# choutilin/makani

Measured on AMD Instinct MI355X. Metric: SFNO fwd+bwd samples/sec, 73ch 721x1440, higher is better.
Workload: dtype bf16; 1 GPU; sfno_linear_73chq_sc3_layers8_edim384 fwd+bwd+Adam, 73ch 721x1440, per-GPU batch 1; global_batch=1, parallelism=h1, spectral_dtype=f32 (GEMMs as 6 bf16 MFMA products of exact 3-way operand splits), step_launch=eager, micro_batches=1, python_gc=disabled in the timed region, adam=after backward

## Files before the change

include/makani_amd.h:

```cpp
#ifndef MAKANI_AMD_H
#define MAKANI_AMD_H

#include <stdint.h>

#ifdef __cplusplus
extern "C" {
#endif

int mk_version(void);
const char* mk_last_error(void);


int mk_quadrature(int grid, int nlat, double* theta, double* weights);

int mk_legendre_kpad(int nlat);

int mk_legendre_table(int grid, int nlat, int lmax, int mmax, int with_quad_weights, float* out);

int mk_fft_twiddle_len(int nlon);
int mk_fft_twiddles(int nlon, float* out);

int mk_rfft(const void* x, int x_dtype, float* xf, const float* twiddles,
            int bc, int nlat, int nlon, int mmax, float scale0, float scale_m, float scale_h,
            void* stream);
// ... 66 lines not shown
int mk_spec_mix_wgrad(const float* x, const float* gy, float* gw, int lloc, int mloc, int batch,
                      int cin, int cout, int l_off, int m_off, void* stream);

int mk_spec_cmlp_fwd(const float* x, const float* w, const float* bias, float* y, int lloc, int mloc, int batch, int cin,
                     int cout, int l_off, int m_off, int per_degree, int act, void* stream);
int mk_spec_cmlp_dgrad(const float* gy, const float* w, const float* a, float* gx, int lloc, int mloc, int batch, int cin,
                       int cout, int l_off, int m_off, int per_degree, int act, void* stream);
long long mk_spec_cmlp_wgrad_workspace(int lloc, int cin, int cout, int per_degree);
int mk_spec_cmlp_wgrad(const float* x, const float* gy, float* gw, void* workspace, int lloc, int mloc, int batch, int cin,
                       int cout, int l_off, int m_off, int per_degree, void* stream);
long long mk_spec_cmlp_bgrad_workspace(int lloc, int cout);
int mk_spec_cmlp_bgrad(const float* g, float* gb, void* workspace, int lloc, int mloc, int batch, int cout, int l_off,
                       int m_off, void* stream);

int mk_spec_bdmlp_fwd(const float* x, const float* w, float* y, int rows, int nb, int ib, int ob, int act, float lambda,
                      void* stream);
int mk_spec_bdmlp_dgrad(const float* gy, const float* w, const float* a, float* gx, int rows, int nb, int ib, int ob, int act,
                        void* stream);
long long mk_spec_bdmlp_wgrad_workspace(int rows, int nb, int ib, int ob);
int mk_spec_bdmlp_wgrad(const float* x, const float* gy, float* gw, void* workspace, int rows, int nb, int ib, int ob,
                        void* stream);
int mk_spec_bdmlp_mask(const float* gy, const float* s, float* out, long long n, void* stream);
int mk_spec_bdmlp_fwd_bias(const float* x, const float* w, const float* bias, float* y, int rows, int nb, int ib, int ob, int act,
                           float lambda, void* stream);

int mk_diag_fwd(const float* x, const float* w, float* y, int batch, int cin, int cout, long long P, void* stream);
int mk_diag_dgrad(const float* gy, const float* w, float* gx, int batch, int cin, int cout, long long P, void* stream);
int mk_diag_wgrad(const float* x, const float* gy, float* gw, int batch, int cin, int cout, long long P, void* stream);

int mk_spec_diag_fwd(const float* x, const float* w, float* y, int lloc, int mloc, int batch,
                     int cin, int cout, int l_off, int m_off, int dense, void* stream);
int mk_spec_diag_dgrad(const float* gy, const float* w, float* gx, int lloc, int mloc, int batch,
                       int cin, int cout, int l_off, int m_off, int dense, void* stream);
int mk_spec_diag_wgrad(const float* x, const float* gy, float* gw, int lloc, int mloc, int batch,
                       int cin, int cout, int l_off, int m_off, int dense, void* stream);

int mk_spec_pack(const float* c_std, float* c_prv, int bc, int lloc, int mloc, void* stream);
int mk_spec_unpack(const float* c_prv, float* c_std, int bc, int lloc, int mloc,
                   int l_off, int m_off, void* stream);
int mk_tokens_to_fields(const void* tok, void* fld, int dtype, int batch, int n, int c, void* stream);
int mk_fields_to_tokens(const void* fld, const void* addend, void* tok, int dtype, int batch, int n, int c, void* stream);
int mk_patch_tile_info(int C, int H, int W, int p0, int p1, int order, long long ldt, int* tile);
int mk_patchify(const void* img, int img_dtype, void* tok, int tok_dtype, long long ldt, int batch, int C, int H, int W, int p0,
                int p1, int order, void* stream);
int mk_unpatchify(const void* tok, int tok_dtype, long long ldt, void* img, int img_dtype, int batch, int C, int H, int W, int p0,
                  int p1, int order, void* stream);

int mk_bias_gelu_fwd(const void* x, const float* bias, void* y, int dtype, int rows, int C, long long P,
                     void* stream);
int mk_bias_gelu_bwd(const void* x, const float* bias, const void* gy, void* gx, float* gbias, int dtype,
                     int rows, int C, long long P, void* stream);
int mk_affine_add(const void* r, const void* z, const float* affine, void* y, int dtype, int rows, long long P,
                  void* stream);
int mk_instnorm_fwd(const void* x, const float* weight, const float* bias, void* y, float* stats,
                    double* workspace, int dtype, int rows, int C, long long P, float eps, int fuse_gelu,
                    void* stream);
int mk_instnorm_bwd(const void* x, const void* gy, const float* stats, const float* weight, const float* bias,
                    void* gx, double* workspace, int dtype, int rows, int C, long long P, int fuse_gelu,
                    void* stream);

int mk_instnorm_fwd_ex(const void* x, const float* weight, const float* bias, void* y, float* stats,
                       double* workspace, int dtype, int rows, int C, long long P, long long count, float eps,
                       int fuse_gelu, int phase, void* stream);
int mk_instnorm_bwd_ex(const void* x, const void* gy, const float* stats, const float* weight, const float* bias,
                       void* gx, double* workspace, int dtype, int rows, int C, long long P, long long count,
                       int fuse_gelu, int phase, void* stream);
int mk_instnorm_bwd_wb(const void* x, const void* gy, const float* stats, const float* weight, const float* bias, void* gx,
                       double* workspace, float* gwb, int dtype, int C, long long P, int fuse_gelu, void* stream);

int mk_wmse_fwd(const void* pred, int dtype, const float* tar, const float* wrow, double* loss, long long rows,
                int H, int W, float scale, void* stream);
int mk_wmse_bwd(const void* pred, int dtype, const float* tar, const float* wrow, const float* gloss, void* gpred,
                long long rows, int H, int W, float scale, void* stream);

int mk_conv1x1_x3(const float* a, long long lda, const float* b, long long ldb, float* c, long long ldc, int M, int K, long long N,
                  int batch, long long sa, long long sb, long long sc, int mode, void* stream);
int mk_conv1x1_x3_bias_act(const float* a, long long lda, const float* b, long long ldb, float* c, long long ldc, int M, int K,
                           long long N, int batch, long long sb, long long sc, const float* bias, int act, void* stream);

int mk_conv1x1_wgrad(const void* gy, const void* x, float* gw, int batch, int cout, int cin, long long P,
                     void* stream);
int mk_conv1x1_wgrad_act(const void* gy, const void* x, float* gw, int batch, int cout, int cin, long long P, int x_act,
                         void* stream);
long long mk_pce_image_bytes(int M, int K);
int mk_pce_pack(const void* w, int w_dtype , int transpose, int M, int K, int ldw, void* img,
                void* stream);
int mk_pce_pack_layout(int M, int K, long long* out3);
int mk_pce_pack_batch(const void* desc_dev, int n, void* arena, long long total_elements, void* stream);
int mk_pce_gemm(const void* x, const void* wimg, void* y, const float* bias, const void* addend, const void* aux_in,
                void* aux_out, int gelu, int batch, int M, int K, long long P, void* stream);
int mk_pce_gemm_ex(const void* x, const void* wimg, void* y, const float* bias, const void* addend, const float* addend_affine,
                   const void* aux_in, void* aux_out, int gelu, double* rowstats, int batch, int M, int K, long long P,
                   void* stream);
long long mk_pce_mlp_image_bytes(int M, int Hd, int K1);
int mk_pce_mlp_pack(const void* a1, int a1_transposed, int lda1, const void* a2, int a2_transposed, int lda2,
                    int w_dtype , int M, int Hd, int K1, void* img, void* stream);
int mk_pce_mlp(const void* x, const void* wimg, void* y, void* mid_out, const void* mid_in, const float* b1, const float* b2,
               double* rowstats_y, double* rowsum_mid, int mode, int batch, int M, int Hd, int K1, long long P, void* stream);
int mk_pce_mlp_debug_stamps(unsigned long long* out512);
int mk_instnorm_coeffs(const double* sums, const float* weight, const float* bias, float* stats, float* affine, int rows,
                       int C, long long count, float eps, void* stream);
int mk_pce_debug_stamps(unsigned long long* out512);

int mk_adam_step(float* p, const float* g, float* m, float* v, long long n, float lr, float beta1, float beta2, float eps,
                 float weight_decay, int step, void* stream);

long long mk_mt_chunks(long long n);
int mk_mt_sumsq(int T, const uint64_t* x, const long long* n, double* partials, double* tsum, int clip_mode, float max_norm,
                float* norm_out, float* coef_out, float* steps, const int* inc_slots, int ninc, void* stream);
int mk_mt_norm_finish(int T, const double* tsum, int clip_mode, float max_norm, float* norm_out, float* coef_out,
                      float* steps, const int* inc_slots, int ninc, void* stream);
int mk_mt_step_inc(float* steps, const int* slots, int nslots, void* stream);
int mk_mt_scale(int T, const uint64_t* x, const long long* n, const float* coef, void* stream);
int mk_mt_adam(int T, const uint64_t* pgmv, const long long* n, const int* step_or_slot, const float* steps, float lr,
               const float* lr_dev, float beta1, float beta2, float eps, float weight_decay, int adamw, const float* coef,
               void* stream);
int mk_mt_lamb(int stage, int T, const uint64_t* pgmv, const long long* n, const int* step_or_slot, const float* steps,
               float lr, const float* lr_dev, float beta1, float beta2, float beta3, float eps, float weight_decay, int adamw,
               int bias_correction, int trust, const float* coef, double* part_p, double* part_u, double* tsum_p,
               double* tsum_u, void* stream);

long long mk_geo_metric_workspace(int B, int C, int H);
int mk_geo_metric_sums(const void* pred, int dtype, const float* tar, const float* clim, const float* wrow, double* workspace,
                       double* sums, int B, int C, int H, int W, void* stream);

long long mk_geo_lp_workspace(int B, int C, int H);
int mk_geo_lp_sums(const void* pred, int dtype, const float* tar, const float* wrow, double* workspace, double* sums, int p,
                   int B, int C, int H, int W, void* stream);
int mk_geo_lp_bwd(const void* pred, int dtype, const float* tar, const float* wrow, const float* g, void* gpred, int p,
                  int B, int C, int H, int W, void* stream);

int mk_input_assemble(const void* x, int x_dtype, const float* u, const float* stat, const float* mean, const float* std,
                      const int* mask_chans, int n_mask, int mask_src, void* out, int out_dtype, int B, int T, int C, int Cu,
                      int Cs, int H, int W, void* stream);
int mk_input_assemble_bwd(const void* gout, int g_dtype, const float* stat, const float* std, const int* mask_chans, int n_mask,
                          int mask_src, void* gx, int x_dtype, int B, int T, int C, int Cu, int Cs, int H, int W, void* stream);

long long mk_history_workspace(int B, int Cn, int H);
int mk_history_sums(const void* x, int x_dtype, const float* u, const float* wt, double* workspace, double* sums, int B, int T,
                    int C, int Cu, int H, int W, void* stream);

long long mk_rollout_tail_workspace(int B, int C, int H);
int mk_rollout_tail(const void* yn, int dtype, const float* mean, const float* std, const float* mask, const int* mask_chans,
                    int n_mask, const float* x_last, long long x_bstride, int residual, const float* scale,
                    const int* hold_chans, int n_hold, float* pred, const float* tar, const float* clim, const float* wrow,
                    double* workspace, double* sums, float* err_map, float* emit, const int* emit_chans, const float* emit_scale,
                    const float* emit_shift, int K, int B, int C, int H, int W, void* stream);

int mk_cos_zenith(const float* eph, const float* sin_lat, const float* cos_lat, const float* lon_rad, float* out, long long n,
                  int H, int W, void* stream);

long long mk_chan_layernorm_workspace(int B, int C, long long P);
int mk_chan_layernorm_fwd(const void* x, int x_dtype, const float* weight, const float* bias, void* y, int y_dtype,
                          float* stats, int B, int C, long long P, float eps, int fuse_gelu, void* stream);
int mk_chan_layernorm_bwd(const void* x, int x_dtype, const void* gy, int gy_dtype, const float* stats, const float* weight,
                          const float* bias, void* gx, float* workspace, float* gwb, int B, int C, long long P, int fuse_gelu,
                          void* stream);

long long mk_degree_power_workspace(int L, int M, int BC);
int mk_degree_power(const float* c, double* workspace, double* P, int L, int M, int BC, int l_off, int m_off, void* stream);
int mk_degree_power_bwd(const float* c, const double* gP, float* gc, int L, int M, int BC, int l_off, int m_off, void* stream);

int mk_attn_info(int D, int* tiles);
int mk_attn_fwd(const void* q, const void* k, const void* v, void* o, float* lse, int B, int H, int Nq, int Nk, int D,
                const long long* strides, float scale, void* stream);
int mk_attn_bwd_delta(const void* o, const void* dO, float* delta, int B, int H, int Nq, int D, const long long* strides,
// ... 52 lines not shown
```

makani_amd/csrc/conv_gemm.hip:

```cpp
#include "common.h"
#include "mfma_tile.h"
#include "../../include/makani_amd.h"
#include "pce_common.h"

#include <hip/hip_bf16.h>
#include <cstdint>
#include <cstdlib>

namespace {

using mk::mfma::bf16x8;
using mk::mfma::f32x16;

__device__ __forceinline__ void act8(uint4& v) {
    uint32_t* w = reinterpret_cast<uint32_t*>(&v);
#pragma unroll
    for (int i = 0; i < 4; ++i) {
        const float lo = __uint_as_float(w[i] << 16), hi = __uint_as_float(w[i] & 0xFFFF0000u);
        w[i] = pce::pack_bf16x2(pce::gelu_f(lo), pce::gelu_f(hi));
    }
}

constexpr int WT = 256;
constexpr int WTI = 128;

struct WgradParams {
    const __hip_bfloat16* gy;
    const __hip_bfloat16* x;
    float* gw;
    int O, I, B;
    long long P;
    int nblk_o, nblk_i, nslab;
    int slab;
    int exp;
};

template <int NV, int WVPR>
__device__ __forceinline__ void wg_load(const __hip_bfloat16* base, long long ld, int rows_valid, long long k0,
                                        long long kend, uint4 (&r)[NV], int tid) {
    typedef unsigned int u4 __attribute__((ext_vector_type(4)));
    const __amdgpu_buffer_rsrc_t rs =
        __builtin_amdgcn_make_buffer_rsrc(const_cast<__hip_bfloat16*>(base), 0, 0x7FFFFFFF, 0x00020000);
#pragma unroll
    for (int i = 0; i < NV; ++i) {
        const int v = tid + i * WT;
        const int row = v / WVPR, c = v % WVPR;
        const long long k = k0 + c * 8;
        const unsigned off = (row < rows_valid && k < kend) ? (unsigned)(((long long)row * ld + k) * 2) : 0x80000000u;
        r[i] = __builtin_bit_cast(uint4, (u4)__builtin_amdgcn_raw_buffer_load_b128(rs, off, 0, 0));
    }
}
template <int NV, int WVPR>
__device__ __forceinline__ void wg_store(char* lds, const uint4 (&r)[NV], int tid) {
    constexpr int WPITCH = WVPR * 16 + 16;
#pragma unroll
    for (int i = 0; i < NV; ++i) {
        const int v = tid + i * WT;
        const int row = v / WVPR, c = v % WVPR;
        *reinterpret_cast<uint4*>(lds + row * WPITCH + c * 16) = r[i];
    }
}

template <int MT, int WTK, int RD = 1, bool ACT = false>
__global__ __launch_bounds__(WT) void conv1x1_wgrad_kernel(WgradParams p) {
    constexpr int WVPR = WTK / 8, WPITCH = WTK * 2 + 16, WTILE_BYTES = WTI * WPITCH;
    constexpr int WTO = 64 * MT, ATILE = WTO * WPITCH, BUF = ATILE + WTILE_BYTES, NVA = WTO * WVPR / WT, NVB = WTI * WVPR / WT;
    extern __shared__ __attribute__((aligned(16))) char lds[];
    const int tid = threadIdx.x, lane = tid & 63, wave = tid >> 6;
    const int wr = wave >> 1, wc = wave & 1;
    const int nblk = p.nblk_o * p.nblk_i;
    const long long bid = blockIdx.x;
    const int xcd = (int)(bid & 7);
    const long long seq = bid >> 3;
    const long long slab_lin = (seq / nblk) * 8 + xcd;
    const int blk = (int)(seq % nblk);
    const long long nslab_tot = (long long)p.nslab * p.B;
    if (slab_lin >= nslab_tot) return;
    const int b = (int)(slab_lin / p.nslab);
    const long long k_begin = (slab_lin % p.nslab) * p.slab;
    const long long k_end = (k_begin + p.slab < p.P) ? k_begin + p.slab : p.P;
    const int o0 = (blk / p.nblk_i) * WTO, i0 = (blk % p.nblk_i) * WTI;
    const __hip_bfloat16* ga = p.gy + ((long long)b * p.O + o0) * p.P;
    const __hip_bfloat16* gb = p.x + ((long long)b * p.I + i0) * p.P;
    const int ov = p.O - o0, iv = p.I - i0;

    f32x16 acc[MT][2];
#pragma unroll
    for (int a = 0; a < MT; ++a)
#pragma unroll
        for (int c = 0; c < 2; ++c)
#pragma unroll
            for (int r = 0; r < 16; ++r) acc[a][c][r] = 0.f;
#pragma unroll
    for (int a = 0; a < MT; ++a)
#pragma unroll
        for (int c = 0; c < 2; ++c) asm volatile("" : "+a"(acc[a][c]));

    uint4 ra[RD][NVA], rb[RD][NVB];
    const int nk = (int)((k_end - k_begin + WTK - 1) / WTK);
    wg_load<NVA, WVPR>(ga, p.P, ov, k_begin, k_end, ra[0], tid);
    wg_load<NVB, WVPR>(gb, p.P, iv, k_begin, k_end, rb[0], tid);
    wg_store<NVA, WVPR>(lds, ra[0], tid);
    if constexpr (ACT) {
#pragma unroll
        for (int i = 0; i < NVB; ++i) act8(rb[0][i]);
    }
    wg_store<NVB, WVPR>(lds + ATILE, rb[0], tid);
#pragma unroll
    for (int d = 0; d < RD; ++d)
        if (d + 1 < nk) {
            const long long k0 = k_begin + (long long)(d + 1) * WTK;
            wg_load<NVA, WVPR>(ga, p.P, ov, k0, k_end, ra[d], tid);
            wg_load<NVB, WVPR>(gb, p.P, iv, k0, k_end, rb[d], tid);
        }
    __syncthreads();
    const int fr = lane & 31, fh = lane >> 5;
    for (int ktb = 0; ktb < nk; ktb += RD) {
#pragma unroll
        for (int d = 0; d < RD; ++d) {
            const int kt = ktb + d;
            if (kt >= nk) break;
            const int cur = kt & 1;
            const char* As = lds + cur * BUF;
            const char* Bs = As + ATILE;
#pragma unroll
            for (int ks = 0; ks < WTK / 16; ++ks) {
                bf16x8 af[MT], bf[2];
#pragma unroll
                for (int a = 0; a < MT; ++a)
                    af[a] = *reinterpret_cast<const bf16x8*>(As + (wr * 32 * MT + a * 32 + fr) * WPITCH + ks * 32 + fh * 16);
#pragma unroll
                for (int c = 0; c < 2; ++c)
                    bf[c] = *reinterpret_cast<const bf16x8*>(Bs + (wc * 64 + c * 32 + fr) * WPITCH + ks * 32 + fh * 16);
#pragma unroll
                for (int a = 0; a < MT; ++a)
#pragma unroll
                    for (int c = 0; c < 2; ++c)
                        acc[a][c] = __builtin_amdgcn_mfma_f32_32x32x16_bf16(af[a], bf[c], acc[a][c], 0, 0, 0);
            }
            if (kt + 1 < nk) {
                wg_store<NVA, WVPR>(lds + (cur ^ 1) * BUF, ra[d], tid);
                if constexpr (ACT) {
#pragma unroll
                    for (int i = 0; i < NVB; ++i) act8(rb[d][i]);
                }
                wg_store<NVB, WVPR>(lds + (cur ^ 1) * BUF + ATILE, rb[d], tid);
                if (kt + 1 + RD < nk) {
                    const long long k0 = k_begin + (long long)(kt + 1 + RD) * WTK;
                    wg_load<NVA, WVPR>(ga, p.P, ov, k0, k_end, ra[d], tid);
                    wg_load<NVB, WVPR>(gb, p.P, iv, k0, k_end, rb[d], tid);
                }
            }
            __syncthreads();
        }
    }
#pragma unroll
    for (int a = 0; a < MT; ++a)
#pragma unroll
        for (int c = 0; c < 2; ++c) {
            const int col = i0 + wc * 64 + c * 32 + fr;
#pragma unroll
            for (int r = 0; r < 16; ++r) {
                const int row = o0 + wr * 32 * MT + a * 32 + (r & 3) + 8 * (r >> 2) + 4 * fh;
                if (row < p.O && col < p.I && (!(p.exp & 1) || acc[a][c][r] == 12345.678f))
                    atomicAdd(&p.gw[(long long)row * p.I + col], acc[a][c][r]);
            }
        }
}



constexpr int WT8 = 512;

template <int NV>
__device__ __forceinline__ void wg8_load(const __hip_bfloat16* base, long long ld, int rows_valid, long long k0,
                                         long long kend, uint4 (&r)[NV], int tid) {
    typedef unsigned int u4 __attribute__((ext_vector_type(4)));
    const __amdgpu_buffer_rsrc_t rs =
        __builtin_amdgcn_make_buffer_rsrc(const_cast<__hip_bfloat16*>(base), 0, 0x7FFFFFFF, 0x00020000);
#pragma unroll
    for (int i = 0; i < NV; ++i) {
        const int v = tid + i * WT8, row = v >> 3, c = v & 7;
        const long long k = k0 + c * 8;
        const unsigned off = (row < rows_valid && k < kend) ? (unsigned)(((long long)row * ld + k) * 2) : 0x80000000u;
        r[i] = __builtin_bit_cast(uint4, (u4)__builtin_amdgcn_raw_buffer_load_b128(rs, off, 0, 0));
    }
}
template <int NV>
__device__ __forceinline__ void wg8_store(char* lds, const uint4 (&r)[NV], int tid) {
#pragma unroll
    for (int i = 0; i < NV; ++i) {
        const int v = tid + i * WT8, row = v >> 3, c = v & 7;
        *reinterpret_cast<uint4*>(lds + row * 144 + c * 16) = r[i];
    }
}

template <int WR, int WC, int RT, int CT, bool ACT = false>
__global__ __launch_bounds__(WT8) void conv1x1_wgrad_big_kernel(WgradParams p) {
    constexpr int TMB = WR * RT * 32, TNB = WC * CT * 32, PITCH = 144;
    constexpr int ATILE = TMB * PITCH, BTILE = TNB * PITCH, BUF = ATILE + BTILE;
    constexpr int NVA = TMB * 8 / WT8, NVB = TNB * 8 / WT8;
    static_assert(WR * WC == 8 && TMB * 8 % WT8 == 0 && TNB * 8 % WT8 == 0, "tile / thread mapping");
    extern __shared__ __attribute__((aligned(16))) char lds[];
    const int tid = threadIdx.x, lane = tid & 63;
    const int wave = __builtin_amdgcn_readfirstlane(tid >> 6);
    const int wr = wave / WC, wc = wave % WC;
    const int nblk = p.nblk_o * p.nblk_i;
    const long long bid = blockIdx.x;
    const int xcd = (int)(bid & 7);
    const long long seq = bid >> 3;
    const long long slab_lin = (seq / nblk) * 8 + xcd;
    const int blk = (int)(seq % nblk);
    const long long nslab_tot = (long long)p.nslab * p.B;
    if (slab_lin >= nslab_tot) return;
    const int b = (int)(slab_lin / p.nslab);
    const long long k_begin = (slab_lin % p.nslab) * p.slab;
    const long long k_end = (k_begin + p.slab < p.P) ? k_begin + p.slab : p.P;
    const int o0 = (blk / p.nblk_i) * TMB, i0 = (blk % p.nblk_i) * TNB;
    const __hip_bfloat16* ga = p.gy + ((long long)b * p.O + o0) * p.P;
    const __hip_bfloat16* gb = p.x + ((long long)b * p.I + i0) * p.P;
    const int ov = p.O - o0, iv = p.I - i0;

    f32x16 acc[RT][CT];
#pragma unroll
    for (int a = 0; a < RT; ++a)
#pragma unroll
        for (int c = 0; c < CT; ++c)
#pragma unroll
            for (int r = 0; r < 16; ++r) acc[a][c][r] = 0.f;
#pragma unroll
    for (int a = 0; a < RT; ++a)
#pragma unroll
        for (int c = 0; c < CT; ++c) asm volatile("" : "+a"(acc[a][c]));

    uint4 ra[NVA], rb[NVB];
    const int nk = (int)((k_end - k_begin + 63) / 64);
    wg8_load<NVA>(ga, p.P, ov, k_begin, k_end, ra, tid);
    wg8_load<NVB>(gb, p.P, iv, k_begin, k_end, rb, tid);
    wg8_store<NVA>(lds, ra, tid);
    if constexpr (ACT) {
#pragma unroll
        for (int i = 0; i < NVB; ++i) act8(rb[i]);
    }
    wg8_store<NVB>(lds + ATILE, rb, tid);
    __syncthreads();
    const int fr = lane & 31, fh = lane >> 5;
    for (int kt = 0; kt < nk; ++kt) {
        const int cur = kt & 1;
        if (kt + 1 < nk) {
            const long long k0 = k_begin + (long long)(kt + 1) * 64;
            wg8_load<NVA>(ga, p.P, ov, k0, k_end, ra, tid);
            wg8_load<NVB>(gb, p.P, iv, k0, k_end, rb, tid);
        }
        const char* As = lds + cur * BUF;
        const char* Bs = As + ATILE;
#pragma unroll
        for (int ks = 0; ks < 4; ++ks) {
            bf16x8 af[RT], bf[CT];
#pragma unroll
            for (int a = 0; a < RT; ++a)
                af[a] = *reinterpret_cast<const bf16x8*>(As + ((wr * RT + a) * 32 + fr) * PITCH + ks * 32 + fh * 16);
#pragma unroll
            for (int c = 0; c < CT; ++c)
                bf[c] = *reinterpret_cast<const bf16x8*>(Bs + ((wc * CT + c) * 32 + fr) * PITCH + ks * 32 + fh * 16);
#pragma unroll
            for (int a = 0; a < RT; ++a)
#pragma unroll
                for (int c = 0; c < CT; ++c)
                    acc[a][c] = __builtin_amdgcn_mfma_f32_32x32x16_bf16(af[a], bf[c], acc[a][c], 0, 0, 0);
        }
        if (kt + 1 < nk) {
            wg8_store<NVA>(lds + (cur ^ 1) * BUF, ra, tid);
            if constexpr (ACT) {
#pragma unroll
                for (int i = 0; i < NVB; ++i) act8(rb[i]);
            }
            wg8_store<NVB>(lds + (cur ^ 1) * BUF + ATILE, rb, tid);
        }
        __syncthreads();
    }
#pragma unroll
    for (int a = 0; a < RT; ++a)
#pragma unroll
        for (int c = 0; c < CT; ++c) {
            const int col = i0 + (wc * CT + c) * 32 + fr;
#pragma unroll
            for (int r = 0; r < 16; ++r) {
                const int row = o0 + (wr * RT + a) * 32 + (r & 3) + 8 * (r >> 2) + 4 * fh;
                if (row < p.O && col < p.I && (!(p.exp & 1) || acc[a][c][r] == 12345.678f))
                    atomicAdd(&p.gw[(long long)row * p.I + col], acc[a][c][r]);
            }
        }
}

}

static void wgrad_slabs(WgradParams& p, long long nblk1, int slots, int batch) {
    long long best_s = 1;
    double best = -1.0;
    for (int w = 1; w <= 4; ++w) {
        const long long sx = ((long long)slots * w) / nblk1;
        if (sx < 1) continue;
        const double score = (double)(sx * nblk1) / ((double)slots * w) - 0.03 * w;
        if (score > best) {
            best = score;
            best_s = sx;
        }
    }
    long long want = (8 * best_s + batch - 1) / batch;
    if (want < 1) want = 1;
    long long slab = (p.P + want - 1) / want;
    slab = (slab + 63) / 64 * 64;
    if (slab < 512) slab = 512;
    p.slab = (int)slab;
    p.nslab = (int)((p.P + p.slab - 1) / p.slab);
}

template <int WR, int WC, int RT, int CT, bool ACT>
static int wgrad_big_launch(WgradParams& p, int batch, hipStream_t st) {
    constexpr int TMB = WR * RT * 32, TNB = WC * CT * 32, LDS = 2 * (TMB + TNB) * 144;
    p.nblk_o = mk::ceil_div(p.O, TMB);
    p.nblk_i = mk::ceil_div(p.I, TNB);
    const long long nblk1 = (long long)p.nblk_o * p.nblk_i;
    wgrad_slabs(p, nblk1, 32, batch);
    const long long grid = (((long long)p.nslab * batch + 7) / 8) * 8 * nblk1;
    MK_REQUIRE_AS("mk_conv1x1_wgrad_act", grid < 2147483647LL, "grid too large");
    MK_REQUIRE_AS("mk_conv1x1_wgrad_act", (mk::raise_lds_limit<conv1x1_wgrad_big_kernel<WR, WC, RT, CT, ACT>>(LDS) == 0),
                  "cannot raise the dynamic LDS limit on this device");
    hipLaunchKernelGGL((conv1x1_wgrad_big_kernel<WR, WC, RT, CT, ACT>), dim3((unsigned)grid), dim3(WT8), LDS, st, p);
    return 0;
}

template <int MT, bool ACT>
static int wgrad_block_launch(WgradParams& p, int batch, hipStream_t st) {
    constexpr int WTO = 64 * MT, LDS = 2 * (WTO + WTI) * (64 * 2 + 16);
    p.nblk_o = mk::ceil_div(p.O, WTO);
    p.nblk_i = mk::ceil_div(p.I, WTI);
    wgrad_slabs(p, (long long)p.nblk_o * p.nblk_i, MT == 4 ? 32 : 64, batch);
    const long long grid = (((long long)p.nslab * batch + 7) / 8) * 8 * p.nblk_o * p.nblk_i;
    MK_REQUIRE_AS("mk_conv1x1_wgrad_act", grid < 2147483647LL, "grid too large");
    MK_REQUIRE_AS("mk_conv1x1_wgrad_act", (mk::raise_lds_limit<conv1x1_wgrad_kernel<MT, 64, 1, ACT>>(LDS) == 0),
                  "cannot raise the dynamic LDS limit on this device");
    hipLaunchKernelGGL((conv1x1_wgrad_kernel<MT, 64, 1, ACT>), dim3((unsigned)grid), dim3(WT), LDS, st, p);
    return 0;
}

extern "C" int mk_conv1x1_wgrad_act(const void* gy, const void* x, float* gw, int batch, int cout, int cin, long long P,
                                    int x_act, void* stream) {
    MK_REQUIRE(gy && x && gw, "null pointer");
    MK_REQUIRE(batch > 0 && cout > 0 && cin > 0 && P > 0, "bad sizes");
    MK_REQUIRE((P % 8) == 0, "P = H*W must be a multiple of 8 (16-byte row alignment)");
    MK_REQUIRE((((uintptr_t)gy | (uintptr_t)x) & 15) == 0, "gy and x must be 16-byte aligned (the tiles are read as uint4)");
    MK_REQUIRE(x_act == 0 || x_act == 1, "x_act must be 0 (none) or 1 (exact GELU)");
    MK_REQUIRE(x_act == 0 || cout <= 384, "the activated operand is built for cout <= 384 (one block row covers all of gy)");
    WgradParams p;
    p.gy = (const __hip_bfloat16*)gy;
    p.x = (const __hip_bfloat16*)x;
    p.gw = gw;
    p.O = cout;
    p.I = cin;
    p.B = batch;
    p.P = P;
    static const int wexp = [] { const char* e = getenv("MK_WGRAD_EXP"); return e ? atoi(e) : 0; }();
    p.exp = wexp;
    hipStream_t st = (hipStream_t)stream;
    int rc;
    if (x_act) {
        if (cout <= 128) rc = wgrad_block_launch<2, true>(p, batch, st);
        else if (cout <= 256) rc = wgrad_block_launch<4, true>(p, batch, st);
        else rc = wgrad_big_launch<4, 2, 3, 2, true>(p, batch, st);
    } else {
        const bool big_ok = P * batch >= 400000;
        if (big_ok && cout % 256 == 0 && cin % 192 == 0) rc = wgrad_big_launch<4, 2, 2, 3, false>(p, batch, st);
        else if (big_ok && cout % 192 == 0 && cin % 256 == 0) rc = wgrad_big_launch<2, 4, 3, 2, false>(p, batch, st);
        else rc = wgrad_block_launch<2, false>(p, batch, st);
    }
    if (rc) return rc;
    MK_LAUNCH_CHECK();
    return 0;
}

extern "C" int mk_conv1x1_wgrad(const void* gy, const void* x, float* gw, int batch, int cout, int cin, long long P,
                                void* stream) {
    return mk_conv1x1_wgrad_act(gy, x, gw, batch, cout, cin, P, 0, stream);
}
```

makani_amd/ops.py:

```python
import ctypes
import math
import os
import typing

import numpy as np
import torch

from . import _lib

GRIDS = {"equiangular": 0, "legendre-gauss": 1}


def _stream():
    return torch.cuda.current_stream().cuda_stream


def _need_cuda(*tensors):
    for t in tensors:
        if not t.is_cuda:
            raise RuntimeError("makani_amd: the spectral ops run only on a HIP device (got a CPU tensor); "
                               "there is no CPU fallback")


def _hip_or_torch(env, default):
# ... 499 lines not shown
        lib = _lib.load()
        rows, self.slots, off, goff = [], {}, 0, 0
        self.gslots = {}
        self.n_fwd = self.total_fwd = 0
        for transpose in (False, True):
            for w in self.weights:
                m, k = (w.shape[1], w.shape[0]) if transpose else (w.shape[0], w.shape[1])
                nbytes = lib.mk_pce_image_bytes(m, k)
                if nbytes <= 0:
                    continue
                lay = (ctypes.c_longlong * 3)()
                _lib.check(lib.mk_pce_pack_layout(m, k, lay), "mk_pce_pack_layout")
                rows.append([w.data_ptr(), 0 if w.dtype == torch.float32 else 1, int(transpose), m, k, w.stride(0), lay[0], lay[1],
                             lay[2], off])
                self.slots[self._key(w, transpose)] = (off * 2, nbytes)
                off += nbytes // 2
            if not transpose:
                self.n_fwd, self.total_fwd = len(rows), off
        for w in self.weights:
            self.gslots[self._key(w, False)] = (goff, w.shape[0], w.shape[1])
            goff += (w.numel() + 3) // 4 * 4
        self.total, self.gtotal = off, goff
        self.n = len(rows)
        dev = self.weights[0].device if self.weights else None
        self.desc = torch.tensor(rows + [[0] * 9 + [off]], dtype=torch.int64).to(dev) if rows else None
        self.images = torch.empty(2 * off, dtype=torch.uint8, device=dev) if rows else None
        self.gbuf = None
        self._prev = None

    @staticmethod
    def _key(w, transpose):
        return (w.data_ptr(), tuple(w.shape), w.stride(0), w.dtype, bool(transpose))

    def refresh(self, with_grad_buffers):
        n, total = (self.n, self.total) if with_grad_buffers else (self.n_fwd, self.total_fwd)
        self._packed_all = bool(with_grad_buffers)
        if n:
            _lib.check(_lib.load().mk_pce_pack_batch(self.desc.data_ptr(), n, self.images.data_ptr(), total, _stream()),
                       "mk_pce_pack_batch")
        self.gbuf = torch.zeros(self.gtotal, dtype=torch.float32, device=self.images.device) if (with_grad_buffers and self.gtotal) else None

    def image(self, w, transpose):
        if transpose and not self._packed_all:
            return None
        slot = self.slots.get(self._key(w, transpose))
        return None if slot is None else self.images[slot[0]:slot[0] + slot[1]]

    def grad_buffer(self, w):
        slot = self.gslots.get(self._key(w, False))
        if slot is None or self.gbuf is None or slot[0] in self._taken:
            return None
        self._taken.add(slot[0])
        return self.gbuf[slot[0]:slot[0] + slot[1] * slot[2]].view(slot[1], slot[2])

    def scope(self):
        return _ArenaScope(self)


class _ArenaScope:
    def __init__(self, arena):
        self.arena = arena

    def __enter__(self):
        global _ACTIVE_ARENA
        self.arena._prev, _ACTIVE_ARENA = _ACTIVE_ARENA, self.arena
        self.arena._taken = set()
        self.arena.refresh(torch.is_grad_enabled())
        return self.arena

    def __exit__(self, *exc):
        global _ACTIVE_ARENA
        _ACTIVE_ARENA = self.arena._prev
        return False


def arena_image(w, transpose=False):
    return None if _ACTIVE_ARENA is None else _ACTIVE_ARENA.image(w, transpose)


def arena_grad_buffer(w):
    return None if _ACTIVE_ARENA is None else _ACTIVE_ARENA.grad_buffer(w)


def conv1x1_wgrad_raw(gy, x3, x_gelu=False, out=None):
    _need_cuda(gy, x3)
    assert gy.is_contiguous() and x3.is_contiguous() and gy.dtype == torch.bfloat16 and x3.dtype == torch.bfloat16
    b, o, p = gy.shape
    i = x3.shape[1]
    if out is not None:
        assert out.dtype == torch.float32 and tuple(out.shape) == (o, i) and out.is_contiguous()
    gw = out if out is not None else torch.zeros(o, i, dtype=torch.float32, device=x3.device)
    _lib.check(_lib.load().mk_conv1x1_wgrad_act(gy.data_ptr(), x3.data_ptr(), gw.data_ptr(), b, o, i, p, int(bool(x_gelu)),
                                                _stream()), "mk_conv1x1_wgrad_act")
    return gw


def pce_supported(m, k):
    return _lib.load().mk_pce_image_bytes(int(m), int(k)) > 0


def pce_supported_train(out_channels, in_channels):
    return pce_supported(out_channels, in_channels) and pce_supported(in_channels, out_channels)


def pce_pack(w, transpose=False):
    _need_cuda(w)
    img = arena_image(w, transpose)
    if img is not None:
        return img
    assert w.dim() == 2 and w.stride(1) == 1 and w.dtype in (torch.float32, torch.bfloat16)
    m, k = (w.shape[1], w.shape[0]) if transpose else (w.shape[0], w.shape[1])
    lib = _lib.load()
    nbytes = lib.mk_pce_image_bytes(m, k)
    if nbytes <= 0:
        raise ValueError(f"pce_pack: unsupported GEMM shape M={m}, K={k}")
    img = torch.empty(nbytes, dtype=torch.uint8, device=w.device)
    _lib.check(lib.mk_pce_pack(w.data_ptr(), 0 if w.dtype == torch.float32 else 1, int(bool(transpose)), m, k, w.stride(0),
                               img.data_ptr(), _stream()), "mk_pce_pack")
    return img


def pce_mlp_supported(m, hd, k1):
    return _lib.load().mk_pce_mlp_image_bytes(int(m), int(hd), int(k1)) > 0


def pce_mlp_pack(a1, a1_transposed, a2, a2_transposed):
    _need_cuda(a1, a2)
    assert a1.dim() == 2 and a2.dim() == 2 and a1.stride(1) == 1 and a2.stride(1) == 1 and a1.dtype == a2.dtype
    assert a1.dtype in (torch.float32, torch.bfloat16)
    hd, k1 = (a1.shape[1], a1.shape[0]) if a1_transposed else (a1.shape[0], a1.shape[1])
    m, hd2 = (a2.shape[1], a2.shape[0]) if a2_transposed else (a2.shape[0], a2.shape[1])
    assert hd == hd2, "the two matrices do not share the hidden dimension"
    lib = _lib.load()
    nbytes = lib.mk_pce_mlp_image_bytes(m, hd, k1)
    if nbytes <= 0:
        raise ValueError(f"pce_mlp_pack: unsupported shape M={m}, Hd={hd}, K1={k1}")
    img = torch.empty(nbytes, dtype=torch.uint8, device=a1.device)
    _lib.check(lib.mk_pce_mlp_pack(a1.data_ptr(), int(bool(a1_transposed)), a1.stride(0), a2.data_ptr(), int(bool(a2_transposed)),
                                   a2.stride(0), 0 if a1.dtype == torch.float32 else 1, m, hd, k1, img.data_ptr(), _stream()),
               "mk_pce_mlp_pack")
    return img, m, hd, k1


def pce_mlp(x3, packed, mode, b1=None, b2=None, pre=None, want_row_sums=False, want_mid_sums=False):
    img, m, hd, k1 = packed
    _need_cuda(x3, img)
    assert x3.dim() == 3 and x3.is_contiguous() and x3.dtype == torch.bfloat16 and x3.shape[1] == k1
    b, _, p = x3.shape
    if mode == 1:
        assert pre is not None and pre.is_contiguous() and pre.dtype == torch.bfloat16 and tuple(pre.shape) == (b, hd, p)
    bf1 = None if b1 is None else b1.detach().float().contiguous()
    bf2 = None if b2 is None else b2.detach().float().contiguous()
    assert (bf1 is None or bf1.numel() == hd) and (bf2 is None or bf2.numel() == m)
    y = torch.empty(b, m, p, dtype=torch.bfloat16, device=x3.device)
    mid = torch.empty(b, hd, p, dtype=torch.bfloat16, device=x3.device)
    sums = torch.empty(b * m, 2, dtype=torch.float64, device=x3.device) if want_row_sums else None
    msum = torch.empty(b * hd, dtype=torch.float64, device=x3.device) if want_mid_sums else None
    _lib.check(_lib.load().mk_pce_mlp(x3.data_ptr(), img.data_ptr(), y.data_ptr(), mid.data_ptr(),
                                      None if pre is None else pre.data_ptr(), None if bf1 is None else bf1.data_ptr(),
                                      None if bf2 is None else bf2.data_ptr(), None if sums is None else sums.data_ptr(),
                                      None if msum is None else msum.data_ptr(), int(mode), b, m, hd, k1, p, _stream()),
               "mk_pce_mlp")
    return (y, mid) + ((sums,) if want_row_sums else ()) + ((msum,) if want_mid_sums else ())


_ZERO_BIAS = {}


def _zero_bias(device):
    z = _ZERO_BIAS.get(device)
    if z is None:
        z = _ZERO_BIAS[device] = torch.zeros(1024, dtype=torch.float32, device=device)
    return z


def pce_gemm(x3, wimg, m, bias=None, addend=None, aux_in=None, want_pre=False, gelu=False, want_row_sums=False,
# ... 2278 lines not shown
```

Before: 23.72 samples/s.

## Add deterministic partial-sum workspace path for 1x1 conv weight gradient

Adds a weight-gradient mode where each K-slab block writes its accumulator tile to a workspace instead of accumulating atomically into gw. A separate sum kernel then reduces the slabs and adds them into gw. The slab-count heuristic is retuned for this mode and the big-tile kernels are enabled at smaller P. The Python side picks this path by default whenever the library reports it is preferred. The cost is extra workspace allocation, extra memory traffic and an extra kernel launch, in exchange for removing atomic contention.

```diff
diff --git a/include/makani_amd.h b/include/makani_amd.h
--- a/include/makani_amd.h
+++ b/include/makani_amd.h
@@ -172,6 +172,10 @@
                      void* stream);
 int mk_conv1x1_wgrad_act(const void* gy, const void* x, float* gw, int batch, int cout, int cin, long long P, int x_act,
                          void* stream);
+int mk_conv1x1_wgrad_prefers_partials(int batch, int cout, int cin, long long P, int x_act);
+long long mk_conv1x1_wgrad_ws_floats(int batch, int cout, int cin, long long P, int x_act);
+int mk_conv1x1_wgrad_ws(const void* gy, const void* x, float* gw, int batch, int cout, int cin, long long P, int x_act,
+                        float* ws, long long ws_floats, void* stream);
 long long mk_pce_image_bytes(int M, int K);
 int mk_pce_pack(const void* w, int w_dtype , int transpose, int M, int K, int ldw, void* img,
                 void* stream);
diff --git a/makani_amd/csrc/conv_gemm.hip b/makani_amd/csrc/conv_gemm.hip
--- a/makani_amd/csrc/conv_gemm.hip
+++ b/makani_amd/csrc/conv_gemm.hip
@@ -33,7 +33,19 @@
     int nblk_o, nblk_i, nslab;
     int slab;
     int exp;
+    float* ws;
 };
+
+template <int NT>
+__device__ __forceinline__ void wg_store_partial(const WgradParams& p, long long slab_lin, int nblk, int blk, int wave, int nwaves,
+                                                 int lane, int t, const f32x16& acc) {
+    float* wp = p.ws + ((slab_lin * nblk + blk) * (long long)(nwaves * NT) + (wave * NT + t)) * 1024 + lane * 4;
+#pragma unroll
+    for (int q = 0; q < 4; ++q) {
+        const float4 v = make_float4(acc[4 * q], acc[4 * q + 1], acc[4 * q + 2], acc[4 * q + 3]);
+        if (!(p.exp & 1) || v.x == 12345.678f) *reinterpret_cast<float4*>(wp + q * 256) = v;
+    }
+}
 
 template <int NV, int WVPR>
 __device__ __forceinline__ void wg_load(const __hip_bfloat16* base, long long ld, int rows_valid, long long k0,
@@ -61,7 +73,7 @@
     }
 }
 
-template <int MT, int WTK, int RD = 1, bool ACT = false>
+template <int MT, int WTK, int RD = 1, bool ACT = false, bool PARTIAL = false>
 __global__ __launch_bounds__(WT) void conv1x1_wgrad_kernel(WgradParams p) {
     constexpr int WVPR = WTK / 8, WPITCH = WTK * 2 + 16, WTILE_BYTES = WTI * WPITCH;
     constexpr int WTO = 64 * MT, ATILE = WTO * WPITCH, BUF = ATILE + WTILE_BYTES, NVA = WTO * WVPR / WT, NVB = WTI * WVPR / WT;
@@ -154,6 +166,13 @@
             __syncthreads();
         }
     }
+    if constexpr (PARTIAL) {
+#pragma unroll
+        for (int a = 0; a < MT; ++a)
+#pragma unroll
+            for (int c = 0; c < 2; ++c) wg_store_partial<MT * 2>(p, slab_lin, nblk, blk, wave, 4, lane, a * 2 + c, acc[a][c]);
+        return;
+    }
 #pragma unroll
     for (int a = 0; a < MT; ++a)
 #pragma unroll
@@ -195,7 +214,7 @@
     }
 }
 
-template <int WR, int WC, int RT, int CT, bool ACT = false>
+template <int WR, int WC, int RT, int CT, bool ACT = false, bool PARTIAL = false>
 __global__ __launch_bounds__(WT8) void conv1x1_wgrad_big_kernel(WgradParams p) {
     constexpr int TMB = WR * RT * 32, TNB = WC * CT * 32, PITCH = 144;
     constexpr int ATILE = TMB * PITCH, BTILE = TNB * PITCH, BUF = ATILE + BTILE;
@@ -279,6 +298,13 @@
         }
         __syncthreads();
     }
+    if constexpr (PARTIAL) {
+#pragma unroll
+        for (int a = 0; a < RT; ++a)
+#pragma unroll
+            for (int c = 0; c < CT; ++c) wg_store_partial<RT * CT>(p, slab_lin, nblk, blk, wave, 8, lane, a * CT + c, acc[a][c]);
+        return;
+    }
 #pragma unroll
     for (int a = 0; a < RT; ++a)
 #pragma unroll
@@ -293,15 +319,71 @@
         }
 }
 
-}
-
-static void wgrad_slabs(WgradParams& p, long long nblk1, int slots, int batch) {
+struct WgradSumParams {
+    const float* ws;
+    float* gw;
+    int O, I, nblk_i;
+    int TM, TN;
+    int NT, CT, WC;
+    long long nslab_tot, img4;
+};
+
+__global__ __launch_bounds__(256) void wgrad_sum_kernel(WgradSumParams s) {
+    const long long g = (long long)blockIdx.x * 256 + threadIdx.x;
+    if (g >= s.img4) return;
+    const float4* src = reinterpret_cast<const float4*>(s.ws) + g;
+    float4 sum = make_float4(0.f, 0.f, 0.f, 0.f);
+    long long t = 0;
+    for (; t + 8 <= s.nslab_tot; t += 8) {
+        float4 v[8];
+#pragma unroll
+        for (int u = 0; u < 8; ++u) v[u] = src[(t + u) * s.img4];
+#pragma unroll
+        for (int u = 0; u < 8; ++u) {
+            sum.x += v[u].x;
+            sum.y += v[u].y;
+            sum.z += v[u].z;
+            sum.w += v[u].w;
+        }
+    }
+    for (; t < s.nslab_tot; ++t) {
+        const float4 v = src[t * s.img4];
+        sum.x += v.x;
+        sum.y += v.y;
+        sum.z += v.z;
+        sum.w += v.w;
+    }
+    const int per_blk4 = s.TM * s.TN / 4;
+    const int blk = (int)(g / per_blk4), rem = (int)(g % per_blk4);
+    const int tile = rem >> 8, q = (rem >> 6) & 3, lane = rem & 63;
+    const int wave = tile / s.NT, tw = tile % s.NT;
+    const int row = (blk / s.nblk_i) * s.TM + ((wave / s.WC) * (s.NT / s.CT) + tw / s.CT) * 32 + 8 * q + 4 * (lane >> 5);
+    const int col = (blk % s.nblk_i) * s.TN + ((wave % s.WC) * s.CT + tw % s.CT) * 32 + (lane & 31);
+    if (col >= s.I) return;
+    const float r[4] = {sum.x, sum.y, sum.z, sum.w};
+#pragma unroll
+    for (int j = 0; j < 4; ++j)
+        if (row + j < s.O) s.gw[(long long)(row + j) * s.I + col] += r[j];
+}
+
+}
+
+enum WgradMode { WG_ATOMIC = 0, WG_PARTIAL = 1, WG_QUERY = 2 };
+struct WgradHost {
+    WgradMode mode;
+    const char* who;
+    long long ws_floats;
+    long long need;
+};
+
+static void wgrad_slabs(WgradParams& p, long long nblk1, int slots, int batch, const WgradHost& h) {
+    const double per_round = h.mode == WG_ATOMIC ? 0.03 : 0.15;
     long long best_s = 1;
     double best = -1.0;
     for (int w = 1; w <= 4; ++w) {
         const long long sx = ((long long)slots * w) / nblk1;
         if (sx < 1) continue;
-        const double score = (double)(sx * nblk1) / ((double)slots * w) - 0.03 * w;
+        const double score = (double)(sx * nblk1) / ((double)slots * w) - per_round * w;
         if (score > best) {
             best = score;
             best_s = sx;
@@ -316,47 +398,102 @@
     p.nslab = (int)((p.P + p.slab - 1) / p.slab);
 }
 
+static int wgrad_workspace(const WgradParams& p, WgradHost& h, int batch, int tm, int tn) {
+    h.need = (long long)p.nslab * batch * p.nblk_o * p.nblk_i * tm * tn;
+    if (h.mode == WG_QUERY) return -1;
+    if (h.mode == WG_PARTIAL) {
+        MK_REQUIRE_AS(h.who, p.ws != nullptr, "null workspace");
+        MK_REQUIRE_AS(h.who, h.ws_floats >= h.need, "workspace too small (mk_conv1x1_wgrad_ws_floats)");
+    }
+    return 0;
+}
+
+static void wgrad_sum_launch(const WgradParams& p, int batch, int tm, int tn, int nt, int ct, int wc, hipStream_t st) {
+    WgradSumParams s;
+    s.ws = p.ws;
+    s.gw = p.gw;
+    s.O = p.O;
+    s.I = p.I;
+    s.nblk_i = p.nblk_i;
+    s.TM = tm;
+    s.TN = tn;
+    s.NT = nt;
+    s.CT = ct;
+    s.WC = wc;
+    s.nslab_tot = (long long)p.nslab * batch;
+    s.img4 = (long long)p.nblk_o * p.nblk_i * tm * tn / 4;
+    hipLaunchKernelGGL(wgrad_sum_kernel, dim3((unsigned)((s.img4 + 255) / 256)), dim3(256), 0, st, s);
+}
+
 template <int WR, int WC, int RT, int CT, bool ACT>
-static int wgrad_big_launch(WgradParams& p, int batch, hipStream_t st) {
+static int wgrad_big_launch(WgradParams& p, int batch, hipStream_t st, WgradHost& h) {
     constexpr int TMB = WR * RT * 32, TNB = WC * CT * 32, LDS = 2 * (TMB + TNB) * 144;
     p.nblk_o = mk::ceil_div(p.O, TMB);
     p.nblk_i = mk::ceil_div(p.I, TNB);
     const long long nblk1 = (long long)p.nblk_o * p.nblk_i;
-    wgrad_slabs(p, nblk1, 32, batch);
+    wgrad_slabs(p, nblk1, 32, batch, h);
+    if (const int w = wgrad_workspace(p, h, batch, TMB, TNB)) return w < 0 ? 0 : w;
     const long long grid = (((long long)p.nslab * batch + 7) / 8) * 8 * nblk1;
-    MK_REQUIRE_AS("mk_conv1x1_wgrad_act", grid < 2147483647LL, "grid too large");
-    MK_REQUIRE_AS("mk_conv1x1_wgrad_act", (mk::raise_lds_limit<conv1x1_wgrad_big_kernel<WR, WC, RT, CT, ACT>>(LDS) == 0),
-                  "cannot raise the dynamic LDS limit on this device");
-    hipLaunchKernelGGL((conv1x1_wgrad_big_kernel<WR, WC, RT, CT, ACT>), dim3((unsigned)grid), dim3(WT8), LDS, st, p);
+    MK_REQUIRE_AS(h.who, grid < 2147483647LL, "grid too large");
+    if (h.mode == WG_PARTIAL) {
+        MK_REQUIRE_AS(h.who, (mk::raise_lds_limit<conv1x1_wgrad_big_kernel<WR, WC, RT, CT, ACT, true>>(LDS) == 0),
+                      "cannot raise the dynamic LDS limit on this device");
+        hipLaunchKernelGGL((conv1x1_wgrad_big_kernel<WR, WC, RT, CT, ACT, true>), dim3((unsigned)grid), dim3(WT8), LDS, st, p);
+        wgrad_sum_launch(p, batch, TMB, TNB, RT * CT, CT, WC, st);
+    } else {
+        MK_REQUIRE_AS(h.who, (mk::raise_lds_limit<conv1x1_wgrad_big_kernel<WR, WC, RT, CT, ACT, false>>(LDS) == 0),
+                      "cannot raise the dynamic LDS limit on this device");
+        hipLaunchKernelGGL((conv1x1_wgrad_big_kernel<WR, WC, RT, CT, ACT, false>), dim3((unsigned)grid), dim3(WT8), LDS, st, p);
+    }
     return 0;
 }
 
 template <int MT, bool ACT>
-static int wgrad_block_launch(WgradParams& p, int batch, hipStream_t st) {
+static int wgrad_block_launch(WgradParams& p, int batch, hipStream_t st, WgradHost& h) {
     constexpr int WTO = 64 * MT, LDS = 2 * (WTO + WTI) * (64 * 2 + 16);
     p.nblk_o = mk::ceil_div(p.O, WTO);
     p.nblk_i = mk::ceil_div(p.I, WTI);
-    wgrad_slabs(p, (long long)p.nblk_o * p.nblk_i, MT == 4 ? 32 : 64, batch);
+    wgrad_slabs(p, (long long)p.nblk_o * p.nblk_i, MT == 4 ? 32 : 64, batch, h);
+    if (const int w = wgrad_workspace(p, h, batch, WTO, WTI)) return w < 0 ? 0 : w;
     const long long grid = (((long long)p.nslab * batch + 7) / 8) * 8 * p.nblk_o * p.nblk_i;
-    MK_REQUIRE_AS("mk_conv1x1_wgrad_act", grid < 2147483647LL, "grid too large");
-    MK_REQUIRE_AS("mk_conv1x1_wgrad_act", (mk::raise_lds_limit<conv1x1_wgrad_kernel<MT, 64, 1, ACT>>(LDS) == 0),
-                  "cannot raise the dynamic LDS limit on this device");
-    hipLaunchKernelGGL((conv1x1_wgrad_kernel<MT, 64, 1, ACT>), dim3((unsigned)grid), dim3(WT), LDS, st, p);
+    MK_REQUIRE_AS(h.who, grid < 2147483647LL, "grid too large");
+    if (h.mode == WG_PARTIAL) {
+        MK_REQUIRE_AS(h.who, (mk::raise_lds_limit<conv1x1_wgrad_kernel<MT, 64, 1, ACT, true>>(LDS) == 0),
+                      "cannot raise the dynamic LDS limit on this device");
+        hipLaunchKernelGGL((conv1x1_wgrad_kernel<MT, 64, 1, ACT, true>), dim3((unsigned)grid), dim3(WT), LDS, st, p);
+        wgrad_sum_launch(p, batch, WTO, WTI, MT * 2, 2, 2, st);
+    } else {
+        MK_REQUIRE_AS(h.who, (mk::raise_lds_limit<conv1x1_wgrad_kernel<MT, 64, 1, ACT, false>>(LDS) == 0),
+                      "cannot raise the dynamic LDS limit on this device");
+        hipLaunchKernelGGL((conv1x1_wgrad_kernel<MT, 64, 1, ACT, false>), dim3((unsigned)grid), dim3(WT), LDS, st, p);
+    }
     return 0;
 }
 
-extern "C" int mk_conv1x1_wgrad_act(const void* gy, const void* x, float* gw, int batch, int cout, int cin, long long P,
-                                    int x_act, void* stream) {
-    MK_REQUIRE(gy && x && gw, "null pointer");
-    MK_REQUIRE(batch > 0 && cout > 0 && cin > 0 && P > 0, "bad sizes");
-    MK_REQUIRE((P % 8) == 0, "P = H*W must be a multiple of 8 (16-byte row alignment)");
-    MK_REQUIRE((((uintptr_t)gy | (uintptr_t)x) & 15) == 0, "gy and x must be 16-byte aligned (the tiles are read as uint4)");
-    MK_REQUIRE(x_act == 0 || x_act == 1, "x_act must be 0 (none) or 1 (exact GELU)");
-    MK_REQUIRE(x_act == 0 || cout <= 384, "the activated operand is built for cout <= 384 (one block row covers all of gy)");
+static long long wgrad_big_from(bool partial) { return partial ? 100000 : 400000; }
+
+extern "C" int mk_conv1x1_wgrad_prefers_partials(int batch, int cout, int cin, long long P, int x_act) {
+    if (x_act || batch <= 0 || P <= 0 || P * batch < wgrad_big_from(true)) return 0;
+    if ((cout % 256 == 0 && cin % 192 == 0) || (cout % 192 == 0 && cin % 256 == 0)) return 1;
+    return P * batch < wgrad_big_from(false) && (long long)mk::ceil_div(cout, 128) * mk::ceil_div(cin, WTI) >= 9;
+}
+
+static int wgrad_run(WgradHost& h, const void* gy, const void* x, float* gw, int batch, int cout, int cin, long long P, int x_act,
+                     float* ws, void* stream) {
+    MK_REQUIRE_AS(h.who, batch > 0 && cout > 0 && cin > 0 && P > 0, "bad sizes");
+    MK_REQUIRE_AS(h.who, (P % 8) == 0, "P = H*W must be a multiple of 8 (16-byte row alignment)");
+    MK_REQUIRE_AS(h.who, x_act == 0 || x_act == 1, "x_act must be 0 (none) or 1 (exact GELU)");
+    MK_REQUIRE_AS(h.who, x_act == 0 || cout <= 384, "the activated operand is built for cout <= 384 (one block row covers all of gy)");
+    if (h.mode != WG_QUERY) {
+        MK_REQUIRE_AS(h.who, gy && x && gw, "null pointer");
+        MK_REQUIRE_AS(h.who, (((uintptr_t)gy | (uintptr_t)x) & 15) == 0, "gy and x must be 16-byte aligned (the tiles are read as uint4)");
+        MK_REQUIRE_AS(h.who, ((uintptr_t)ws & 15) == 0, "the workspace must be 16-byte aligned");
+    }
     WgradParams p;
     p.gy = (const __hip_bfloat16*)gy;
     p.x = (const __hip_bfloat16*)x;
     p.gw = gw;
+    p.ws = ws;
     p.O = cout;
     p.I = cin;
     p.B = batch;
@@ -366,21 +503,39 @@
     hipStream_t st = (hipStream_t)stream;
     int rc;
     if (x_act) {
-        if (cout <= 128) rc = wgrad_block_launch<2, true>(p, batch, st);
-        else if (cout <= 256) rc = wgrad_block_launch<4, true>(p, batch, st);
-        else rc = wgrad_big_launch<4, 2, 3, 2, true>(p, batch, st);
+        if (cout <= 128) rc = wgrad_block_launch<2, true>(p, batch, st, h);
+        else if (cout <= 256) rc = wgrad_block_launch<4, true>(p, batch, st, h);
+        else rc = wgrad_big_launch<4, 2, 3, 2, true>(p, batch, st, h);
     } else {
-        const bool big_ok = P * batch >= 400000;
-        if (big_ok && cout % 256 == 0 && cin % 192 == 0) rc = wgrad_big_launch<4, 2, 2, 3, false>(p, batch, st);
-        else if (big_ok && cout % 192 == 0 && cin % 256 == 0) rc = wgrad_big_launch<2, 4, 3, 2, false>(p, batch, st);
-        else rc = wgrad_block_launch<2, false>(p, batch, st);
+        const bool big_ok = P * batch >= wgrad_big_from(h.mode != WG_ATOMIC);
+        if (big_ok && cout % 256 == 0 && cin % 192 == 0) rc = wgrad_big_launch<4, 2, 2, 3, false>(p, batch, st, h);
+        else if (big_ok && cout % 192 == 0 && cin % 256 == 0) rc = wgrad_big_launch<2, 4, 3, 2, false>(p, batch, st, h);
+        else rc = wgrad_block_launch<2, false>(p, batch, st, h);
     }
     if (rc) return rc;
-    MK_LAUNCH_CHECK();
+    if (h.mode != WG_QUERY) MK_LAUNCH_CHECK_AS(h.who);
     return 0;
+}
+
+extern "C" int mk_conv1x1_wgrad_act(const void* gy, const void* x, float* gw, int batch, int cout, int cin, long long P,
+                                    int x_act, void* stream) {
+    WgradHost h{WG_ATOMIC, __func__, 0, 0};
+    return wgrad_run(h, gy, x, gw, batch, cout, cin, P, x_act, nullptr, stream);
 }
 
 extern "C" int mk_conv1x1_wgrad(const void* gy, const void* x, float* gw, int batch, int cout, int cin, long long P,
                                 void* stream) {
-    return mk_conv1x1_wgrad_act(gy, x, gw, batch, cout, cin, P, 0, stream);
-}
+    WgradHost h{WG_ATOMIC, __func__, 0, 0};
+    return wgrad_run(h, gy, x, gw, batch, cout, cin, P, 0, nullptr, stream);
+}
+
+extern "C" long long mk_conv1x1_wgrad_ws_floats(int batch, int cout, int cin, long long P, int x_act) {
+    WgradHost h{WG_QUERY, __func__, 0, 0};
+    return wgrad_run(h, nullptr, nullptr, nullptr, batch, cout, cin, P, x_act, nullptr, nullptr) ? -1 : h.need;
+}
+
+extern "C" int mk_conv1x1_wgrad_ws(const void* gy, const void* x, float* gw, int batch, int cout, int cin, long long P, int x_act,
+                                   float* ws, long long ws_floats, void* stream) {
+    WgradHost h{WG_PARTIAL, __func__, ws_floats, 0};
+    return wgrad_run(h, gy, x, gw, batch, cout, cin, P, x_act, ws, stream);
+}
diff --git a/makani_amd/ops.py b/makani_amd/ops.py
--- a/makani_amd/ops.py
+++ b/makani_amd/ops.py
@@ -605,6 +605,15 @@
     return None if _ACTIVE_ARENA is None else _ACTIVE_ARENA.grad_buffer(w)
 
 
+def _wgrad_partials(b, o, i, p, x_gelu):
+    mode = os.environ.get("MK_WGRAD_COMBINE")
+    if mode is None:
+        return bool(_lib.load().mk_conv1x1_wgrad_prefers_partials(b, o, i, p, int(bool(x_gelu))))
+    if mode not in ("partials", "atomic"):
+        raise ValueError(f"unknown MK_WGRAD_COMBINE {mode!r} (partials | atomic)")
+    return mode == "partials"
+
+
 def conv1x1_wgrad_raw(gy, x3, x_gelu=False, out=None):
     _need_cuda(gy, x3)
     assert gy.is_contiguous() and x3.is_contiguous() and gy.dtype == torch.bfloat16 and x3.dtype == torch.bfloat16
@@ -613,8 +622,15 @@
     if out is not None:
         assert out.dtype == torch.float32 and tuple(out.shape) == (o, i) and out.is_contiguous()
     gw = out if out is not None else torch.zeros(o, i, dtype=torch.float32, device=x3.device)
-    _lib.check(_lib.load().mk_conv1x1_wgrad_act(gy.data_ptr(), x3.data_ptr(), gw.data_ptr(), b, o, i, p, int(bool(x_gelu)),
-                                                _stream()), "mk_conv1x1_wgrad_act")
+    lib = _lib.load()
+    if _wgrad_partials(b, o, i, p, x_gelu):
+        n = lib.mk_conv1x1_wgrad_ws_floats(b, o, i, p, int(bool(x_gelu)))
+        ws = torch.empty(max(n, 0), dtype=torch.float32, device=x3.device)
+        _lib.check(lib.mk_conv1x1_wgrad_ws(gy.data_ptr(), x3.data_ptr(), gw.data_ptr(), b, o, i, p, int(bool(x_gelu)), ws.data_ptr(),
+                                           ws.numel(), _stream()), "mk_conv1x1_wgrad_ws")
+        return gw
+    _lib.check(lib.mk_conv1x1_wgrad_act(gy.data_ptr(), x3.data_ptr(), gw.data_ptr(), b, o, i, p, int(bool(x_gelu)),
+                                        _stream()), "mk_conv1x1_wgrad_act")
     return gw
 
 
```

Measured after the change: 23.89 samples/s, median of 6. Within noise of the previous version (+0.7%).
